# numamma/numamma

Measured on AMD Instinct MI355X. Metric: PEBS samples/s analysed (device-resident), higher is better.
Workload: dtype u64

## Files before the change

### numamma_amd/csrc/nmg_engine_impl.h

```cpp
#pragma once

#include <dlfcn.h>
#include <hip/hip_runtime.h>
#include <rccl/rccl.h>
#include <rocprofiler-sdk-roctx/roctx.h>

#include <algorithm>
#include <chrono>
#include <cinttypes>
#include <functional>
#include <cstdio>
#include <cstdlib>
#include <cstddef>
#include <cstring>
#include <condition_variable>
#include <memory>
#include <mutex>
#include <string>
#include <thread>
#include <vector>

#include "nmg_buffer.h"
#include "nmg_kernels.h"
#include "nmg_route.h"
// ... 70 lines not shown
  DevBuf<DevEntry> own_chain;
  DevEntry* chain = nullptr;
  uint32_t K = 0, elevels = 0, nb_fences = 0, fence_log2 = 0, dir_log2 = 0;
};

struct RouteTable {
  bool ok = false;
  uint32_t nparts = 0;
  DevBuf<PartInfo> d_parts;
  DevBuf<uint64_t> d_pbounds;
  DevBuf<uint16_t> d_pdir;
  DevBuf<uint32_t> d_pdead;
  DevBuf<uint64_t> d_pe_keys;
  DevBuf<uint4> d_pe_nodes;
  DevBuf<uint4> d_pe_pnode;
  DevBuf<uint4> d_pe_old;
  DevBuf<uint32_t> d_pe_oinf;
  DevBuf<uint2> d_pe_info;
  DevBuf<uint4> d_pe_dir;
  DevBuf<uint32_t> d_pe_ids;
  DevBuf<uint32_t> d_pe_lrel;
  DevBuf<uint32_t> d_pe_cmap;
};

struct RoutePool {
  DevBuf<uint4> d_rec16;
  DevBuf<uint32_t> d_cmeta;
  DevBuf<unsigned long long> d_cmatch;
  DevBuf<uint32_t> d_clist;
  DevBuf<uint4> d_items;
  DevBuf<uint32_t> d_chunk0;
  DevBuf<uint32_t> d_used;
  DevBuf<uint32_t> d_pcnt;
  DevBuf<uint32_t> d_pbase;
  DevBuf<uint32_t> d_ctl;
  DevBuf<uint4> d_ovf16;
  DevBuf<unsigned long long> d_ovfx;
};

struct EntryTable {
  std::vector<uint64_t> hist_base;
  std::vector<uint64_t> npages;
  std::vector<uint64_t> buffer_size, entry_addr;
  std::vector<nmg_object> objects;
  std::vector<DevEntry> dev_entries;
  std::vector<uint32_t> sparse_entries;
  CellCursor cur;

  uint64_t cells() const { return cur.cells; }
  void resize(uint32_t E) {
    const size_t E0 = dev_entries.size();
    hist_base.resize(E, kHistSparse);
    npages.resize(E, 1);
    buffer_size.resize(E, 0);
    entry_addr.resize(E, 0);
    objects.resize(E, nmg_object{0, 0, 0, 0});
    dev_entries.resize(E, DevEntry{0, 0, 0, 0, kHistSparse, ~0u, 0, 0, 0, 0});
    for (size_t e = E0; e < E; e++) dev_entries[e].id = (uint32_t)e;
  }
  void truncate(uint32_t E, const CellCursor& c) {
    resize(E);
    sparse_entries.resize(c.nsparse);
    cur = c;
  }
  void describe(uint32_t id, const nmg_object& o) {
    objects[id] = o;
    buffer_size[id] = o.buffer_size;
    entry_addr[id] = o.buffer_addr;
// ... 276 lines not shown
```

### numamma_amd/csrc/nmg_route.h

```cpp
#pragma once

#include "nmg_kernels.h"

namespace nmg {

constexpr uint32_t kChunk = 64;
constexpr uint32_t kPartLevels = 11;
constexpr uint32_t kMaxParts = (1u << kPartLevels) - 1;
constexpr uint32_t kRouteDir = 4096;
constexpr uint32_t kRouteSegs = 8;
constexpr uint32_t kDirCntSat = 31;
struct RSeg {
  uint64_t start;
  uint32_t base;
  uint32_t nslots;
  uint32_t shift;
  uint32_t qlast;
};
constexpr uint32_t kPartKeys = 1023;
constexpr uint32_t kPartSlots = 1024;
constexpr uint32_t kPartDir = 1024;
constexpr uint32_t kDirInline = 6;
constexpr uint32_t kPnQShift = 8;
constexpr uint32_t kPnOlder = 1u << 11, kPnExact = 1u << 12;
// ... 29 lines not shown
  uint32_t pages_lds;
  uint32_t cmap;
  uint32_t pad[2];
};
static_assert(sizeof(PartInfo) == 48, "PartInfo");

constexpr uint32_t kAddrBits = 40;
constexpr uint32_t kMinWeightBits = 11;
constexpr uint32_t kTsBits = 40;
struct XLayout {
  uint32_t gbits, obits, tbits, wbits;
  uint64_t wesc;
  uint64_t tbase;
};

struct RouteParams {
  Params p;
  const uint64_t* pbounds;
  const uint16_t* pdir;
  const uint32_t* pdead;
  RSeg seg[kRouteSegs];
  uint32_t nseg;
  uint32_t nparts;
  XLayout xl;
  uint64_t seq0;
  uint4* rec16;
  uint32_t* cmeta;
  const uint32_t* chunk0;
  uint32_t* used;
  uint4* ovf16;
  unsigned long long* ovfx;
  uint32_t* ovf_cnt;
  uint32_t ovf_cap;
};

struct PlanParams {
  uint32_t* pcnt;
  uint32_t* pbase;
  uint4* items;
  uint32_t* ctl;
  uint32_t grid, nparts;
};

struct ScatterParams {
  const uint32_t* cmeta;
  const uint32_t* chunk0;
  const uint32_t* used;
  const uint32_t* pcnt;
  const uint32_t* pbase;
  uint32_t* clist;
  uint32_t nparts;
};

struct LocalParams {
  Params p;
  const PartInfo* parts;
  const uint64_t* pe_keys;
  const uint4* pe_nodes;
  const uint4* pe_pnode;
  const uint4* pe_old;
  const uint32_t* pe_oinf;
  const uint2* pe_info;
  const uint4* pe_dir;
  const uint32_t* pe_ids;
  const uint32_t* pe_lrel;
  const uint32_t* pe_cmap;
  const uint4* rec16;
  const uint32_t* cmeta;
  const uint32_t* clist;
  const uint4* items;
  uint32_t* ctl;
  unsigned long long* cmatch;
  const BufDesc* descs;
  XLayout xl;
  uint64_t seq0;
  uint32_t fresh;
};

struct FoundParams {
  const uint32_t* ranges;
  const uint32_t* chunk0;
  const uint32_t* used;
  const uint32_t* cmeta;
  const unsigned long long* cmatch;
  const uint4* rec16;
  uint32_t* bufcnt;
  uint32_t nb_bufs, gbits, gshift;
};

hipError_t launch_route(uint32_t grid, hipStream_t s, const RouteParams& r);
hipError_t launch_overflow(hipStream_t s, const RouteParams& r);
struct CountParams {
  ScatterParams sc;
};
hipError_t launch_count(uint32_t grid, hipStream_t s, const CountParams& r);
hipError_t launch_plan(hipStream_t s, const PlanParams& r);
hipError_t launch_scatter(uint32_t grid, hipStream_t s, const ScatterParams& r);
hipError_t launch_local(uint32_t grid, hipStream_t s, const LocalParams& r);
hipError_t launch_found(uint32_t grid, hipStream_t s, const FoundParams& r);

}
```

### numamma_amd/csrc/nmg_route.hip

```cpp
#include <algorithm>

#include "nmg_device.h"
#include "nmg_route.h"

namespace nmg {

static_assert((uint64_t)kItemChunks * kChunk * kLaneMaxWeight < (1ull << kPackShift), "packed weight per item");


struct XRec {
  uint64_t addr, ts, w;
  uint64_t loc;
  uint32_t th, acc;
  bool esc;
  __device__ __forceinline__ uint32_t g(const XLayout& xl) const { return uint32_t(loc >> xl.obits); }
  __device__ __forceinline__ uint32_t off(const XLayout& xl) const {
    return uint32_t(loc & ((1ull << xl.obits) - 1)) << 3;
  }
};

__device__ __forceinline__ uint4 x_encode(const XLayout& xl, uint64_t pb, uint64_t addr, uint64_t ts, uint64_t w,
                                          uint32_t g, uint32_t off, uint32_t th, uint32_t acc) {
  const uint64_t ar = addr - pb, tr = ts - xl.tbase;
  const bool fit = (ar >> kAddrBits) == 0 && ts >= xl.tbase && (tr >> kTsBits) == 0 && w < xl.wesc;
// ... 321 lines not shown
__device__ __forceinline__ Claim route2_settle(uint64_t old, uint32_t q, unsigned long long* s_state, uint32_t& taken,
                                               uint32_t capl, uint32_t* cmeta, uint32_t c0) {
  Claim r;
  r.dst = ~0ull;
  r.lid = 0;
  r.waitg = 0;
  r.ovf = false;
  r.ok = true;
  const uint32_t f = st_cnt(old), g = st_gen(old), cu = st_cur(old), nx = st_next(old);
  if (cu != kStNone && f < 2 * kChunk) {
    const uint32_t c = f < kChunk ? cu : nx;
    if (c == kStOvf) r.ovf = true;
    else r.dst = uint64_t(c0 + c) * kChunk + (f & (kChunk - 1));
    r.lid = ((g << 6) + f) >> 2;
    if (f == kChunk + kChunk / 2) {
      const uint32_t n2 = route2_take(taken, capl);
      if (n2 != kStOvf) cmeta[c0 + n2] = q | (kChunk << 24);
      route2_advance(&s_state[q], g, n2, n2, false, old + 1);
    }
  } else if (cu == kStNone && f == 2 * kChunk) {
    const uint32_t n1 = route2_take(taken, capl);
    const uint32_t n2 = n1 == kStOvf ? kStOvf : route2_take(taken, capl);
    if (n1 != kStOvf) cmeta[c0 + n1] = q | (kChunk << 24);
    if (n2 != kStOvf) cmeta[c0 + n2] = q | (kChunk << 24);
    route2_advance(&s_state[q], g, n1, n2, true, old + 1);
    if (n1 == kStOvf) r.ovf = true;
    else r.dst = uint64_t(c0 + n1) * kChunk;
    r.lid = (g + 1) << 4;
  } else {
    r.waitg = g;
    r.ok = false;
  }
  return r;
}

struct XF {
  uint4 a;
  uint32_t q;
  uint32_t lvl;
  bool routed;
};

template <bool TIMING>
__global__ __launch_bounds__(kR2WG, 1) void route2_kernel(RouteParams rp) {
  __shared__ uint64_t s_pb[kMaxParts + 1];
  __shared__ uint16_t s_pdir[kRouteDir];
  __shared__ uint32_t s_dead[(kMaxParts + 1) / 32];
  __shared__ unsigned long long s_state[kMaxParts + 1];
  __shared__ uint4 s_desc[kDescLds];
  __shared__ uint32_t s_wlist[kWaves][64];
  __shared__ uint32_t s_taken, s_bnext;
  __shared__ unsigned long long s_gsums[2][kGlobalSums], s_gmins[2][kBuckets], s_gmaxs[2][kBuckets];
  __shared__ SegL s_seg[kRouteSegs];
  __shared__ uint64_t s_segst[kRouteSegs];
  __shared__ uint4 s_line[kLineParts * 4];
  __shared__ LineWord s_lw[kLineParts];
  __shared__ uint32_t s_ldst[kLineParts];
  __shared__ uint2 s_tab[kWaves][64];

  Params& p = rp.p;
  const int tid = threadIdx.x;
  const int lane = tid & 63, wave = tid >> 6;
  if (tid < (int)kRouteSegs) {
    const RSeg g = rp.seg[tid];
    s_seg[tid].a = make_uint4((uint32_t)g.start, (uint32_t)(g.start >> 32), g.base, g.nslots);
    s_seg[tid].b = make_uint4(g.shift, g.qlast, 0, 0);
// ... 320 lines not shown
            if (xr.esc) x_resolve(xr, rp.xl, p.data, p.sbufs);
            direct_attribute(p, xr.addr, xr.ts, xr.w, xr.th, xr.acc, X.lvl, rp.seq0 + xr.g(rp.xl), xr.off(rp.xl),
                             xr.g(rp.xl));
          }
        }
        vm_drain();
      }
      rt_stamp<TIMING>(rt, 10);
    };

    XF X;
    do {
      front(ra, rb, X);
      back(X);
      front(rb, ra, X);
      back(X);
    } while (d0.pad != kNoBuf);

    if (TIMING && lane == 0) {
      unsigned long long* o = p.dbg + (uint64_t(blockIdx.x) * (kWG / 64) + tid / 64) * kRouteTimingWords;
      for (int k = 0; k < 9; k++) o[k] = rt.acc[k];
      o[9] = nwin;
      uint32_t nb = 0;
      if (wave == 0)
        for (uint32_t q = 0; q < nlp; q++) nb += (s_lw[q] & kLwBroken) ? 1u : 0u;
      o[10] = nb;
      o[11] = rt.acc[9];
      o[12] = rt.acc[10];
    }
  }
  racc_drain(gacc[0], s_gsums[0], lane);
  racc_drain(gacc[1], s_gsums[1], lane);
  lds_sync();
#pragma unroll
  for (uint32_t a = 0; a < 2; a++) {
    if (tid < (int)kGlobalSums && s_gsums[a][tid])
      atomicAdd(reinterpret_cast<unsigned long long*>(p.sum64 + gsum_index(a, tid)), s_gsums[a][tid]);
    if (tid < (int)kBuckets && s_gsums[a][3 + 2 * tid]) {
      atomicMin(reinterpret_cast<unsigned long long*>(p.min64 + a * kBuckets + tid), s_gmins[a][tid]);
      atomicMax(reinterpret_cast<unsigned long long*>(p.max64 + a * kBuckets + tid), s_gmaxs[a][tid]);
    }
  }
  for (uint32_t q = tid; q < P; q += kR2WG) {
    const unsigned long long st = s_state[q];
    const uint32_t f = st_cnt(st), cu = st_cur(st), nx = st_next(st);
    if (cu == kStNone) continue;
    if (cu != kStOvf) rp.cmeta[c0 + cu] = q | (min(f, kChunk) << 24);
    if (nx != kStOvf) rp.cmeta[c0 + nx] = q | ((f > kChunk ? f - kChunk : 0u) << 24);
    if (q < nlp) {
      const uint32_t m = lw_mask(s_lw[q]);
      for (uint32_t j = 0; j < 4; j++)
        if ((m >> j) & 1u) rp.rec16[uint64_t(s_ldst[q]) * 4 + j] = s_line[q * 4 + j];
    }
  }
  if (tid == 0) rp.used[blockIdx.x] = min(s_taken, capl);
}


__global__ __launch_bounds__(256) void overflow_kernel(RouteParams rp) {
  const uint32_t n = min(*rp.ovf_cnt, rp.ovf_cap);
  for (uint32_t i = blockIdx.x * 256 + threadIdx.x; i < n; i += gridDim.x * 256) {
    XRec xr = x_decode(rp.xl, rp.ovfx[i], rp.ovf16[i]);
    if (xr.esc) x_resolve(xr, rp.xl, rp.p.data, rp.p.sbufs);
    const uint32_t lvl = (rp.p.flags & NMG_F_OBJECT_LEVELS)
                             ? raw_mem_lvl(rp.p.data, rp.p.sbufs[xr.g(rp.xl)].offset + xr.off(rp.xl))
                             : 0u;
    direct_attribute(rp.p, xr.addr, xr.ts, xr.w, xr.th, xr.acc, lvl, rp.seq0 + xr.g(rp.xl), xr.off(rp.xl),
                     xr.g(rp.xl));
  }
}


__global__ __launch_bounds__(kWG) void count_kernel(CountParams cp) {
  __shared__ uint32_t s_cnt[kMaxParts + 1];
  const ScatterParams& r = cp.sc;
  const uint32_t tid = threadIdx.x, w = blockIdx.x, P = r.nparts;
  for (uint32_t q = tid; q < P; q += kWG) s_cnt[q] = 0;
  __syncthreads();
  const uint32_t c0 = r.chunk0[w], n = r.used[w];
  constexpr uint32_t kU = 8;
  for (uint32_t b = 0; b < n; b += kU * kWG) {
    uint32_t m[kU];
#pragma unroll
    for (uint32_t u = 0; u < kU; u++) {
      const uint32_t i = b + u * kWG + tid;
      m[u] = i < n ? r.cmeta[c0 + i] : 0u;
    }
#pragma unroll
    for (uint32_t u = 0; u < kU; u++)
      if (m[u] >> 24) atomicAdd(&s_cnt[m[u] & 0xffffffu], 1u);
  }
  __syncthreads();
  uint32_t* out = const_cast<uint32_t*>(r.pcnt) + uint64_t(w) * P;
  for (uint32_t q = tid; q < P; q += kWG) out[q] = s_cnt[q];
}

constexpr uint32_t kPlanRowGroups = kWG / 64;
__global__ __launch_bounds__(kWG) void plan_cols_kernel(PlanParams r) {
  __shared__ uint32_t s_sum[kPlanRowGroups][64];
  const uint32_t tid = threadIdx.x, c = tid & 63, rg = tid >> 6;
  const uint32_t P = r.nparts, q = blockIdx.x * 64 + c;
  const uint32_t per = (r.grid + kPlanRowGroups - 1) / kPlanRowGroups, w0 = rg * per;
  constexpr uint32_t kU = 16;
  uint32_t sum = 0;
  for (uint32_t b = 0; b < per; b += kU) {
    uint32_t v[kU];
#pragma unroll
    for (uint32_t u = 0; u < kU; u++) {
      const uint32_t w = w0 + b + u;
      v[u] = (q < P && b + u < per && w < r.grid) ? r.pcnt[uint64_t(w) * P + q] : 0u;
    }
#pragma unroll
    for (uint32_t u = 0; u < kU; u++) sum += v[u];
  }
  s_sum[rg][c] = sum;
  __syncthreads();
  uint32_t run = 0;
  for (uint32_t g = 0; g < rg; g++) run += s_sum[g][c];
  for (uint32_t b = 0; b < per; b += kU) {
    uint32_t v[kU];
#pragma unroll
    for (uint32_t u = 0; u < kU; u++) {
      const uint32_t w = w0 + b + u;
      v[u] = (q < P && b + u < per && w < r.grid) ? r.pcnt[uint64_t(w) * P + q] : 0u;
    }
#pragma unroll
    for (uint32_t u = 0; u < kU; u++) {
      const uint32_t w = w0 + b + u;
      if (q < P && b + u < per && w < r.grid) r.pcnt[uint64_t(w) * P + q] = run;
      run += v[u];
    }
  }
  if (q < P && rg == kPlanRowGroups - 1) r.pbase[q] = run;
}

__global__ __launch_bounds__(kWG) void plan_kernel(PlanParams r) {
  __shared__ uint32_t s_tot[kMaxParts + 1], s_nit[kMaxParts + 1], s_wsum[2][kWG / 64];
  const int tid = threadIdx.x, lane = tid & 63, wave = tid >> 6;
  const uint32_t P = r.nparts;
  for (uint32_t q = tid; q < P; q += kWG) {
    const uint32_t run = r.pbase[q];
    s_tot[q] = run;
    s_nit[q] = (run + kItemChunks - 1) / kItemChunks;
  }
  __syncthreads();
  const uint32_t i0 = 2 * (uint32_t)tid;
  const uint32_t t0 = i0 < P ? s_tot[i0] : 0u, t1 = i0 + 1 < P ? s_tot[i0 + 1] : 0u;
  const uint32_t n0 = i0 < P ? s_nit[i0] : 0u, n1 = i0 + 1 < P ? s_nit[i0 + 1] : 0u;
  uint32_t it = t0 + t1, in = n0 + n1;
#pragma unroll
  for (int o = 1; o < 64; o <<= 1) {
    const uint32_t a = __shfl_up(it, o, 64), b = __shfl_up(in, o, 64);
    if (lane >= o) {
      it += a;
      in += b;
    }
  }
  if (lane == 63) {
    s_wsum[0][wave] = it;
    s_wsum[1][wave] = in;
  }
  __syncthreads();
  uint32_t wt = 0, wn = 0;
  for (int w2 = 0; w2 < wave; w2++) {
    wt += s_wsum[0][w2];
    wn += s_wsum[1][w2];
  }
  const uint32_t tb = wt + it - (t0 + t1), nb = wn + in - (n0 + n1);
  for (uint32_t k = 0; k < 2; k++) {
    const uint32_t q = i0 + k;
    if (q >= P) break;
    const uint32_t base = tb + (k ? t0 : 0u), ibase = nb + (k ? n0 : 0u), tot = k ? t1 : t0;
    r.pbase[q] = base;
    for (uint32_t j = 0; j * kItemChunks < tot; j++)
      r.items[ibase + j] = make_uint4(q, base + j * kItemChunks, base + min(tot, (j + 1) * kItemChunks),
                                      tot <= kItemChunks ? 1u : 0u);
  }
  if (tid == kWG - 1) {
    r.ctl[0] = wn + in;
    r.ctl[1] = 0;
    r.ctl[3] = r.ctl[2];
    r.ctl[2] = 0;
  }
}

__global__ __launch_bounds__(kWG) void scatter_kernel(ScatterParams r) {
  __shared__ uint32_t s_cnt[kMaxParts + 1];
  const uint32_t tid = threadIdx.x, w = blockIdx.x, P = r.nparts;
  const uint32_t* off = r.pcnt + uint64_t(w) * P;
  for (uint32_t q = tid; q < P; q += kWG) s_cnt[q] = r.pbase[q] + off[q];
  __syncthreads();
  const uint32_t c0 = r.chunk0[w], n = r.used[w];
  constexpr uint32_t kU = 8;
  for (uint32_t b = 0; b < n; b += kU * kWG) {
    uint32_t m[kU];
#pragma unroll
    for (uint32_t u = 0; u < kU; u++) {
      const uint32_t i = b + u * kWG + tid;
      m[u] = i < n ? r.cmeta[c0 + i] : 0u;
    }
#pragma unroll
    for (uint32_t u = 0; u < kU; u++) {
      if (!(m[u] >> 24)) continue;
      const uint32_t k = atomicAdd(&s_cnt[m[u] & 0xffffffu], 1u);
      r.clist[k] = (c0 + b + u * kWG + tid) | ((m[u] >> 24) << kChunkIdBits);
    }
  }
}


constexpr uint32_t kLWG = 1024;
constexpr int kLC = 2;

template <typename T>
__device__ __forceinline__ T l2_load(const T* p) {
  return __hip_atomic_load(p, __ATOMIC_RELAXED, __HIP_MEMORY_SCOPE_AGENT);
}

__device__ __forceinline__ uint64_t entry_id(const LocalParams& lp, uint32_t pos) {
  return lp.pe_ids ? lp.pe_ids[pos] : pos;
}

__device__ __forceinline__ int32_t match_older_pos(const Params& p, uint32_t first, uint32_t count, uint64_t addr,
                                                   uint64_t ts, uint64_t& baddr, uint64_t& hist) {
  for (uint32_t j = first + 1; j < first + count; j++) {
    const uint4* r = reinterpret_cast<const uint4*>(p.chain + j);
    const uint4 ra = r[0], rb = r[1];
    if (entry_match(ra, rb, addr, ts)) {
      const uint4 rc = r[2];
      baddr = u64of(ra.x, ra.y);
      hist = u64of(rc.x, rc.y);
      return (int32_t)j;
    }
  }
  return -1;
}

template <bool TIMING, bool PACKED, bool EXTRA>
__global__ __launch_bounds__(kLWG, 1) void local_kernel(LocalParams lp) {
  __shared__ uint64_t s_keys[kPartSlots];
  __shared__ uint4 s_pn[kPartSlots];
  __shared__ uint2 s_info[kPartSlots];
  __shared__ uint4 s_dir[kPartDir];
  __shared__ uint4 s_old[kOldLds];
  __shared__ uint32_t s_oinf[kOldLds];
  __shared__ unsigned long long s_owt[2][kPartEntries];
  __shared__ unsigned long long s_first[kPartEntries];
  __shared__ uint32_t s_pg[kPartCells / 2];
  __shared__ uint32_t s_clist[kItemChunks];
  __shared__ uint32_t s_item, s_cnext, s_nfound, s_big, s_took;
// ... 414 lines not shown
        if (TIMING) {
          const uint64_t now = stamp();
          textra += now - rt.last;
          rt.last = now;
        }
      }
    };
    uint4 A[kLC], B[kLC];
    auto grab = [&]() -> uint32_t {
      uint32_t t = 0;
      if (lane == 0) t = atomicAdd(&s_cnext, (uint32_t)kLC);
      return __builtin_amdgcn_readfirstlane(t);
    };
    uint32_t la = grab(), lb = grab();
#pragma unroll
    for (int j = 0; j < kLC; j++) chunk_load(la + j, A[j]);
#pragma unroll
    for (int j = 0; j < kLC; j++) chunk_load(lb + j, B[j]);
    while (la < nl) {
      process(la, A);
      la = grab();
#pragma unroll
      for (int j = 0; j < kLC; j++) chunk_load(la + j, A[j]);
      if (lb < nl) process(lb, B);
      lb = grab();
#pragma unroll
      for (int j = 0; j < kLC; j++) chunk_load(lb + j, B[j]);
    }
    uint32_t won = 0;
    if (lane == 0) won = atomicExch(&s_took, 1u) == 0 ? 1u : 0u;
    if (__builtin_amdgcn_readfirstlane(won)) take_next();
    lds_sync();
    rt_stamp<TIMING>(rt, 9);
    const bool clean =excl && lp.fresh && __builtin_amdgcn_readfirstlane(lp.ctl[3]) == 0;
    const bool clean_obj = clean && __builtin_amdgcn_readfirstlane(s_big) == 0;
    for (uint32_t i = tid; i < pi.ne; i += kLWG) {
      const uint64_t e = entry_id(lp, pi.e0 + i);
#pragma unroll
      for (uint32_t a = 0; a < 2; a++) {
        const uint64_t v = s_owt[a][i];
        if (!v) continue;
        s_owt[a][i] = 0;
        const uint64_t cnt = v >> kPackShift, wt = v & ((1ull << kPackShift) - 1);
        uint64_t* pc = p.sum64 + objcw_index(e, a, 0, p.nb_entries);
        uint64_t* pw = p.sum64 + objcw_index(e, a, 1, p.nb_entries);
        if (clean_obj) {
          *pc = cnt;
          if (wt) *pw = wt;
        } else if (excl) {
          *pc = l2_load(pc) + cnt;
          if (wt) *pw = l2_load(pw) + wt;
        } else {
          atomicAdd(reinterpret_cast<unsigned long long*>(pc), (unsigned long long)cnt);
          if (wt) atomicAdd(reinterpret_cast<unsigned long long*>(pw), (unsigned long long)wt);
        }
      }
      const uint64_t floc = s_first[i];
      if (floc != ~0ull) {
        s_first[i] = ~0ull;
        const uint64_t fo = ((lp.seq0 + (floc >> lp.xl.obits)) << 32) | ((floc & ((1ull << lp.xl.obits) - 1)) << 3);
        uint64_t* pf = p.min64 + kFirstBase + e;
        if (clean) *pf = fo;
        else if (excl) *pf = min(l2_load(pf), fo);
        else atomicMin(reinterpret_cast<unsigned long long*>(pf), (unsigned long long)fo);
      }
    }
    {
// ... 56 lines not shown
  for (uint32_t i = tid; i < nl; i += kWG) s_found[i] = 0;
  __syncthreads();
  const uint64_t k0 = uint64_t(r.chunk0[w]) * kChunk, k1 = k0 + uint64_t(r.used[w]) * kChunk;
  const uint64_t gmask = (1ull << r.gbits) - 1;
  constexpr int kU = 4;
  for (uint64_t k = k0 + tid; k < k1; k += kU * kWG) {
    uint64_t bits[kU], xw[kU];
#pragma unroll
    for (int u = 0; u < kU; u++) {
      const uint64_t kk = k + u * kWG;
      bits[u] = kk < k1 && (r.cmeta[kk / kChunk] >> 24) ? r.cmatch[kk / kChunk] : 0ull;
      xw[u] = ((bits[u] >> lane) & 1) ? reinterpret_cast<const uint64_t*>(r.rec16)[2 * kk + 1] >> r.gshift : 0ull;
    }
#pragma unroll
    for (int u = 0; u < kU; u++) {
      if (!((bits[u] >> lane) & 1)) continue;
      const uint32_t g = (uint32_t)(xw[u] & gmask);
      if (g - g0 < nl) atomicAdd(&s_found[g - g0], 1u);
      else atomicAdd(r.bufcnt + r.nb_bufs + g, 1u);
    }
  }
  __syncthreads();
  for (uint32_t i = tid; i < nl; i += kWG)
    if (s_found[i]) atomicAdd(r.bufcnt + r.nb_bufs + g0 + i, s_found[i]);
}


hipError_t launch_route(uint32_t grid, hipStream_t s, const RouteParams& r) {
  if (r.p.flags & kDbgRouteTiming) hipLaunchKernelGGL(route2_kernel<true>, dim3(grid), dim3(kR2WG), 0, s, r);
  else hipLaunchKernelGGL(route2_kernel<false>, dim3(grid), dim3(kR2WG), 0, s, r);
  return hipGetLastError();
}

hipError_t launch_plan(hipStream_t s, const PlanParams& r) {
  if (r.nparts) hipLaunchKernelGGL(plan_cols_kernel, dim3((r.nparts + 63) / 64), dim3(kWG), 0, s, r);
  hipLaunchKernelGGL(plan_kernel, dim3(1), dim3(kWG), 0, s, r);
  return hipGetLastError();
}

hipError_t launch_overflow(hipStream_t s, const RouteParams& r) {
  hipLaunchKernelGGL(overflow_kernel, dim3(1024), dim3(256), 0, s, r);
  return hipGetLastError();
}

hipError_t launch_count(uint32_t grid, hipStream_t s, const CountParams& r) {
  hipLaunchKernelGGL(count_kernel, dim3(grid), dim3(kWG), 0, s, r);
  return hipGetLastError();
}

hipError_t launch_scatter(uint32_t grid, hipStream_t s, const ScatterParams& r) {
  hipLaunchKernelGGL(scatter_kernel, dim3(grid), dim3(kWG), 0, s, r);
  return hipGetLastError();
}

template <bool TIMING, bool PACKED>
static void launch_local_as(bool extra, uint32_t grid, hipStream_t s, const LocalParams& r) {
  if (extra) hipLaunchKernelGGL((local_kernel<TIMING, PACKED, true>), dim3(grid), dim3(kLWG), 0, s, r);
  else hipLaunchKernelGGL((local_kernel<TIMING, PACKED, false>), dim3(grid), dim3(kLWG), 0, s, r);
}

hipError_t launch_local(uint32_t grid, hipStream_t s, const LocalParams& r) {
  const bool timing = (r.p.flags & kDbgLocalTiming) != 0, packed = r.pe_cmap != nullptr;
  const bool extra = (r.p.flags & NMG_F_OBJECT_LEVELS) != 0 || r.p.smatch != nullptr;
  if (packed) {
    if (timing) launch_local_as<true, true>(extra, grid, s, r);
    else launch_local_as<false, true>(extra, grid, s, r);
  } else {
    if (timing) launch_local_as<true, false>(extra, grid, s, r);
    else launch_local_as<false, false>(extra, grid, s, r);
  }
  return hipGetLastError();
}

hipError_t launch_found(uint32_t grid, hipStream_t s, const FoundParams& r) {
  hipLaunchKernelGGL(found_kernel, dim3(grid), dim3(kWG), 0, s, r);
  return hipGetLastError();
}

}
```

### numamma_amd/csrc/nmg_route_host.hip

```cpp
#include "nmg_engine_impl.h"


uint32_t bits_for(uint64_t v) {
  uint32_t b = 0;
  while (b < 64 && (v >> b) != 0) b++;
  return b;
}

bool route_layout(nmg_engine* h, const std::vector<BufDesc>& descs, XLayout& xl) {
  uint64_t maxlen = 1;
  for (const BufDesc& d : descs) maxlen = std::max<uint64_t>(maxlen, d.len);
  xl.gbits = bits_for(descs.size() - 1);
  xl.obits = bits_for((maxlen - 1) / 8);
  xl.tbits = bits_for(h->T - 1);
  const uint32_t loc = xl.gbits + xl.obits + xl.tbits + 1;
  if (loc > 48 - kMinWeightBits || xl.gbits > 31 || xl.obits > 31 || xl.tbits > 31) return false;
  xl.wbits = std::min<uint32_t>(48 - loc, 16);
  xl.wesc = (1ull << xl.wbits) - 1;
  xl.tbase = h->route_tbase;
  return true;
}

bool route_eligible(nmg_engine* h, const std::vector<BufDesc>& descs) {
  constexpr uint32_t kLegacyOnly = kDbgLoadOnly | kDbgNoGlobal | kDbgNoFlush | kDbgNoTables | kDbgTiming |
// ... 12 lines not shown
bool route_eligible(nmg_engine* h) { return route_eligible(h, h->descs); }

int route_pool(nmg_engine* h, const std::vector<BufDesc>& descs, uint32_t grid, const uint32_t* ranges,
                      std::vector<uint32_t>& c0) {
  const uint32_t P = h->rt.nparts;
  c0.assign(grid + 1, 0);
  uint64_t tot = 0;
  for (uint32_t w = 0; w < grid; w++) {
    uint64_t rec = 0;
    for (uint32_t b = ranges[w]; b < ranges[w + 1]; b++) rec += (descs[b].len + kRecBytes - 1) / kRecBytes;
    const uint64_t cap = (h->flags & kDbgTinyPool) ? 2 : (rec + kChunk - 1) / kChunk + 2 * P;
    c0[w] = (uint32_t)tot;
    tot += cap;
  }
  c0[grid] = (uint32_t)tot;
  if (tot >= (1ull << kChunkIdBits)) return fail(h, NMG_ERR_RANGE, "partition-first chunk pool too large");
  const size_t items = tot / kItemChunks + P + 1;
  uint64_t recs = 0;
  for (const BufDesc& d : descs) recs += (d.len + kRecBytes - 1) / kRecBytes;
  const size_t ovf = (size_t)((h->flags & kDbgTinyPool) ? recs : recs / 4 + std::min<uint64_t>(3 * recs, 4u << 20)) + 65536;
  RoutePool& rp = h->rpool;
  if (tot > rp.d_cmeta.cap() || items > rp.d_items.cap() || grid > rp.d_used.cap() || ovf > rp.d_ovfx.cap()) {
    HIP_TRY(h, hipStreamSynchronize(h->stream));
    rp = RoutePool();
    const size_t cap = std::max<size_t>(tot, 1);
    HIP_TRY(h, rp.d_rec16.alloc(cap * kChunk));
    HIP_TRY(h, rp.d_cmeta.alloc(cap));
    HIP_TRY(h, rp.d_cmatch.alloc(cap));
    HIP_TRY(h, rp.d_clist.alloc(cap));
    HIP_TRY(h, rp.d_items.alloc(items));
    HIP_TRY(h, rp.d_chunk0.alloc(grid + 1));
    HIP_TRY(h, rp.d_used.alloc(grid));
    HIP_TRY(h, rp.d_pcnt.alloc((size_t)grid * (kMaxParts + 1)));
    HIP_TRY(h, rp.d_pbase.alloc(kMaxParts + 1));
    HIP_TRY(h, rp.d_ctl.alloc(4));
    HIP_TRY(h, hipMemset(rp.d_ctl, 0, 4 * 4));
    HIP_TRY(h, rp.d_ovf16.alloc(ovf));
    HIP_TRY(h, rp.d_ovfx.alloc(ovf));
  }
  return NMG_OK;
}

int route_prepare(nmg_engine* h, uint32_t grid, const std::vector<uint32_t>& ranges) {
  std::vector<uint32_t> c0;
  const int rc = route_pool(h, h->descs, grid, ranges.data(), c0);
  if (rc) return rc;
  const int rc2 = stage_h2d(h, h->rpool.d_chunk0, c0.data(), (grid + 1) * 4);
  if (rc2) return rc2;
  h->route_sched_key = h->rt.nparts | ((h->flags & kDbgTinyPool) ? 0x80000000u : 0u);
  return NMG_OK;
}


int route_analyze(nmg_engine* h, uint32_t nb, uint32_t grid) {
  (void)nb;
  RouteJob job{&h->descs, h->d_data, h->d_sdescs, h->d_ranges, h->rpool.d_chunk0, grid, 0, false};
  return route_analyze_job(h, job);
}

int route_analyze_job(nmg_engine* h, const RouteJob& job) {
  Range range("nmg_route");
  XLayout xl;
  if (!route_layout(h, *job.descs, xl)) return fail(h, NMG_ERR_STATE, "route layout");
  const uint32_t grid = job.grid;
  Params base = base_params(h, job.data, job.sdescs, job.ranges);
  base.bufcnt = h->d_bufcnt + job.index_base;
  const uint64_t seq0 = (*job.descs)[0].seq;
  h->route_launches++;
  int slot = 0;
  int rc = launch_events(h, &slot);
  if (rc) return rc;
  HIP_TRY(h, hipEventRecord(h->ring0[slot], h->stream));
  RouteParams rp;
  memset(&rp, 0, sizeof(rp));
  rp.p = base;
  rp.pbounds = h->rt.d_pbounds;
  rp.pdir = h->rt.d_pdir;
  rp.pdead = h->rt.d_pdead;
  for (uint32_t k = 0; k < kRouteSegs; k++) rp.seg[k] = h->rsegs[k];
  rp.nseg = h->nrsegs;
  rp.nparts = h->rt.nparts;
  rp.xl = xl;
  rp.seq0 = seq0;
  rp.rec16 = h->rpool.d_rec16;
  rp.cmeta = h->rpool.d_cmeta;
  rp.chunk0 = job.chunk0;
  rp.used = h->rpool.d_used;
  rp.ovf16 = h->rpool.d_ovf16;
  rp.ovfx = h->rpool.d_ovfx;
  rp.ovf_cnt = h->rpool.d_ctl + 2;
  rp.ovf_cap = (uint32_t)std::min<size_t>(h->rpool.d_ovfx.cap(), 0xffffffffu);
  if (h->flags & kDbgTinyOvf) rp.ovf_cap = std::min<uint32_t>(rp.ovf_cap, 64);
  if (h->flags & kDbgRouteTiming) {
    rc = ensure_dbg(h, (size_t)grid * (kWG / 64) * kRouteTimingWords);
    if (rc) return rc;
    rp.p.dbg = reinterpret_cast<unsigned long long*>(h->d_dbg.get());
  }
  HIP_TRY(h, launch_route(grid, h->stream, rp));
  HIP_TRY(h, hipEventRecord(h->ringr[slot], h->stream));
  HIP_TRY(h, launch_overflow(h->stream, rp));
  ScatterParams sc;
  sc.cmeta = h->rpool.d_cmeta;
  sc.chunk0 = job.chunk0;
  sc.used = h->rpool.d_used;
  sc.pcnt = h->rpool.d_pcnt;
  sc.pbase = h->rpool.d_pbase;
  sc.clist = h->rpool.d_clist;
  sc.nparts = h->rt.nparts;
  CountParams cp;
  memset(&cp, 0, sizeof(cp));
  cp.sc = sc;
  HIP_TRY(h, launch_count(grid, h->stream, cp));
  PlanParams pl;
  pl.pcnt = h->rpool.d_pcnt;
  pl.pbase = h->rpool.d_pbase;
  pl.items = h->rpool.d_items;
  pl.ctl = h->rpool.d_ctl;
  pl.grid = grid;
  pl.nparts = h->rt.nparts;
  HIP_TRY(h, launch_plan(h->stream, pl));
  HIP_TRY(h, launch_scatter(grid, h->stream, sc));
  LocalParams lp;
  memset(&lp, 0, sizeof(lp));
  lp.p = base;
  lp.parts = h->rt.d_parts;
  lp.pe_keys = h->rt.d_pe_keys;
  lp.pe_nodes = h->rt.d_pe_nodes;
  lp.pe_info = h->rt.d_pe_info;
  lp.pe_pnode = h->rt.d_pe_pnode;
  lp.pe_old = h->rt.d_pe_old;
  lp.pe_oinf = h->rt.d_pe_oinf;
  lp.pe_dir = h->rt.d_pe_dir;
  lp.pe_ids = h->rt.d_pe_ids;
  lp.pe_lrel = h->rt.d_pe_lrel;
  lp.pe_cmap = h->rt.d_pe_cmap;
  lp.rec16 = h->rpool.d_rec16;
  lp.cmeta = h->rpool.d_cmeta;
  lp.clist = h->rpool.d_clist;
  lp.items = h->rpool.d_items;
  lp.ctl = h->rpool.d_ctl;
  lp.cmatch = h->rpool.d_cmatch;
  lp.descs = job.sdescs;
  lp.xl = xl;
  lp.seq0 = seq0;
  lp.fresh = h->counters_fresh ? 1u : 0u;
  h->counters_fresh = false;
  if ((h->flags & kDbgLocalTiming) && !(h->flags & kDbgRouteTiming)) {
    rc = ensure_dbg(h, (size_t)h->num_cus * (kWG / 64) * kRouteTimingWords);
    if (rc) return rc;
    lp.p.dbg = reinterpret_cast<unsigned long long*>(h->d_dbg.get());
  }
  HIP_TRY(h, launch_local((uint32_t)h->num_cus, h->stream, lp));
  HIP_TRY(h, hipEventRecord(h->ringm[slot], h->stream));
  HIP_TRY(h, hipEventRecord(h->ring1[slot], h->stream));
  h->nlaunch++;
  h->launched = true;
  if (job.settle_now) {
    FoundParams f;
    f.ranges = job.ranges;
    f.chunk0 = job.chunk0;
    f.used = h->rpool.d_used;
    f.cmeta = h->rpool.d_cmeta;
    f.cmatch = h->rpool.d_cmatch;
    f.rec16 = h->rpool.d_rec16;
    f.bufcnt = h->d_bufcnt + job.index_base;
    f.nb_bufs = (uint32_t)h->bufcnt_stride;
    f.gbits = xl.gbits;
    f.gshift = 16 + xl.wbits + xl.obits;
    HIP_TRY(h, launch_found(grid, h->stream, f));
    return NMG_OK;
  }
  h->route_pending = true;
  h->route_grid = grid;
// ... 23 lines not shown
```

Before: 45.76 billion.

## Fold count and plan into route/scatter kernels with atomic partition totals

The route kernel now counts per-partition chunks itself, right after writing cmeta, and reserves per-block offsets with agent-scope atomic adds on a partition-total array. The scatter kernel absorbs the overflow handling, the item-plan scan and the per-block base computation, so four separate launches (overflow, count, plan_cols, plan) disappear. Double-buffered totals and overflow counters, selected by launch parity, are reset for the next launch from inside scatter. The cost is that per-block offsets now depend on atomic ordering instead of a deterministic column scan. It also adds redundant scan work in every scatter block and a cmeta re-read with a drain and barrier in route.

```diff
diff --git a/numamma_amd/csrc/nmg_engine_impl.h b/numamma_amd/csrc/nmg_engine_impl.h
--- a/numamma_amd/csrc/nmg_engine_impl.h
+++ b/numamma_amd/csrc/nmg_engine_impl.h
@@ -126,8 +126,9 @@
   DevBuf<uint32_t> d_chunk0;
   DevBuf<uint32_t> d_used;
   DevBuf<uint32_t> d_pcnt;
-  DevBuf<uint32_t> d_pbase;
+  DevBuf<uint32_t> d_ptot;
   DevBuf<uint32_t> d_ctl;
+  uint32_t launches = 0;
   DevBuf<uint4> d_ovf16;
   DevBuf<unsigned long long> d_ovfx;
 };
diff --git a/numamma_amd/csrc/nmg_route.h b/numamma_amd/csrc/nmg_route.h
--- a/numamma_amd/csrc/nmg_route.h
+++ b/numamma_amd/csrc/nmg_route.h
@@ -85,14 +85,8 @@
   unsigned long long* ovfx;
   uint32_t* ovf_cnt;
   uint32_t ovf_cap;
-};
-
-struct PlanParams {
+  uint32_t* ptot;
   uint32_t* pcnt;
-  uint32_t* pbase;
-  uint4* items;
-  uint32_t* ctl;
-  uint32_t grid, nparts;
 };
 
 struct ScatterParams {
@@ -100,8 +94,12 @@
   const uint32_t* chunk0;
   const uint32_t* used;
   const uint32_t* pcnt;
-  const uint32_t* pbase;
+  const uint32_t* ptot;
+  uint32_t* ptot_next;
+  uint32_t* ovf_next;
   uint32_t* clist;
+  uint4* items;
+  uint32_t* ctl;
   uint32_t nparts;
 };
 
@@ -123,6 +121,7 @@
   const uint32_t* clist;
   const uint4* items;
   uint32_t* ctl;
+  const uint32_t* ovf_cnt;
   unsigned long long* cmatch;
   const BufDesc* descs;
   XLayout xl;
@@ -142,13 +141,7 @@
 };
 
 hipError_t launch_route(uint32_t grid, hipStream_t s, const RouteParams& r);
-hipError_t launch_overflow(hipStream_t s, const RouteParams& r);
-struct CountParams {
-  ScatterParams sc;
-};
-hipError_t launch_count(uint32_t grid, hipStream_t s, const CountParams& r);
-hipError_t launch_plan(hipStream_t s, const PlanParams& r);
-hipError_t launch_scatter(uint32_t grid, hipStream_t s, const ScatterParams& r);
+hipError_t launch_scatter(uint32_t grid, hipStream_t s, const RouteParams& r, const ScatterParams& sc);
 hipError_t launch_local(uint32_t grid, hipStream_t s, const LocalParams& r);
 hipError_t launch_found(uint32_t grid, hipStream_t s, const FoundParams& r);
 
diff --git a/numamma_amd/csrc/nmg_route.hip b/numamma_amd/csrc/nmg_route.hip
--- a/numamma_amd/csrc/nmg_route.hip
+++ b/numamma_amd/csrc/nmg_route.hip
@@ -377,6 +377,11 @@
     r.ok = false;
   }
   return r;
+}
+
+template <typename T>
+__device__ __forceinline__ T l2_load(const T* p) {
+  return __hip_atomic_load(p, __ATOMIC_RELAXED, __HIP_MEMORY_SCOPE_AGENT);
 }
 
 struct XF {
@@ -763,6 +768,8 @@
   racc_drain(gacc[0], s_gsums[0], lane);
   racc_drain(gacc[1], s_gsums[1], lane);
   lds_sync();
+  uint32_t* s_cnt = reinterpret_cast<uint32_t*>(s_pb);
+  for (uint32_t q = tid; q < P; q += kR2WG) s_cnt[q] = 0;
 #pragma unroll
   for (uint32_t a = 0; a < 2; a++) {
     if (tid < (int)kGlobalSums && s_gsums[a][tid])
@@ -784,13 +791,37 @@
         if ((m >> j) & 1u) rp.rec16[uint64_t(s_ldst[q]) * 4 + j] = s_line[q * 4 + j];
     }
   }
-  if (tid == 0) rp.used[blockIdx.x] = min(s_taken, capl);
-}
-
-
-__global__ __launch_bounds__(256) void overflow_kernel(RouteParams rp) {
-  const uint32_t n = min(*rp.ovf_cnt, rp.ovf_cap);
-  for (uint32_t i = blockIdx.x * 256 + threadIdx.x; i < n; i += gridDim.x * 256) {
+  const uint32_t nused = __builtin_amdgcn_readfirstlane(min(s_taken, capl));
+  if (tid == 0) rp.used[blockIdx.x] = nused;
+  vm_drain();
+  __syncthreads();
+  constexpr uint32_t kTU = 4;
+  for (uint32_t b = 0; b < nused; b += kTU * kR2WG) {
+    uint32_t m[kTU];
+#pragma unroll
+    for (uint32_t u = 0; u < kTU; u++) {
+      const uint32_t i = b + u * kR2WG + tid;
+      m[u] = i < nused ? l2_load(rp.cmeta + c0 + i) : 0u;
+    }
+#pragma unroll
+    for (uint32_t u = 0; u < kTU; u++)
+      if (m[u] >> 24) atomicAdd(&s_cnt[m[u] & 0xffffffu], 1u);
+  }
+  lds_sync();
+  uint32_t* out = rp.pcnt + uint64_t(blockIdx.x) * P;
+  for (uint32_t q = tid; q < P; q += kR2WG) {
+    const uint32_t n = s_cnt[q];
+    out[q] = n ? __hip_atomic_fetch_add(rp.ptot + q, n, __ATOMIC_RELAXED, __HIP_MEMORY_SCOPE_AGENT) : 0u;
+  }
+}
+
+static_assert(2 * kWG >= kMaxParts + 1, "scatter_kernel scans two partitions per thread");
+__global__ __launch_bounds__(kWG) void scatter_kernel(RouteParams rp, ScatterParams r) {
+  __shared__ uint32_t s_cnt[kMaxParts + 1];
+  __shared__ uint32_t s_wsum[2][kWG / 64];
+  const uint32_t tid = threadIdx.x, lane = tid & 63, wave = tid >> 6, w = blockIdx.x, P = r.nparts;
+  const uint32_t novf = min(*rp.ovf_cnt, rp.ovf_cap);
+  for (uint32_t i = w * kWG + tid; i < novf; i += gridDim.x * kWG) {
     XRec xr = x_decode(rp.xl, rp.ovfx[i], rp.ovf16[i]);
     if (xr.esc) x_resolve(xr, rp.xl, rp.p.data, rp.p.sbufs);
     const uint32_t lvl = (rp.p.flags & NMG_F_OBJECT_LEVELS)
@@ -799,14 +830,50 @@
     direct_attribute(rp.p, xr.addr, xr.ts, xr.w, xr.th, xr.acc, lvl, rp.seq0 + xr.g(rp.xl), xr.off(rp.xl),
                      xr.g(rp.xl));
   }
-}
-
-
-__global__ __launch_bounds__(kWG) void count_kernel(CountParams cp) {
-  __shared__ uint32_t s_cnt[kMaxParts + 1];
-  const ScatterParams& r = cp.sc;
-  const uint32_t tid = threadIdx.x, w = blockIdx.x, P = r.nparts;
-  for (uint32_t q = tid; q < P; q += kWG) s_cnt[q] = 0;
+  const uint32_t* off = r.pcnt + uint64_t(w) * P;
+  const uint32_t i0 = 2 * tid;
+  const uint32_t t0 = i0 < P ? r.ptot[i0] : 0u, t1 = i0 + 1 < P ? r.ptot[i0 + 1] : 0u;
+  const uint32_t o0 = i0 < P ? off[i0] : 0u, o1 = i0 + 1 < P ? off[i0 + 1] : 0u;
+  const uint32_t n0 = (t0 + kItemChunks - 1) / kItemChunks, n1 = (t1 + kItemChunks - 1) / kItemChunks;
+  uint32_t it = t0 + t1, in = n0 + n1;
+#pragma unroll
+  for (int o = 1; o < 64; o <<= 1) {
+    const uint32_t a = __shfl_up(it, o, 64), b = __shfl_up(in, o, 64);
+    if (lane >= (uint32_t)o) {
+      it += a;
+      in += b;
+    }
+  }
+  if (lane == 63) {
+    s_wsum[0][wave] = it;
+    s_wsum[1][wave] = in;
+  }
+  __syncthreads();
+  uint32_t wt = 0, wn = 0;
+  for (uint32_t w2 = 0; w2 < wave; w2++) {
+    wt += s_wsum[0][w2];
+    wn += s_wsum[1][w2];
+  }
+  const uint32_t tb = wt + it - (t0 + t1), nb = wn + in - (n0 + n1);
+  if (i0 < P) s_cnt[i0] = tb + o0;
+  if (i0 + 1 < P) s_cnt[i0 + 1] = tb + t0 + o1;
+  if (w == 0) {
+    for (uint32_t k = 0; k < 2; k++) {
+      const uint32_t q = i0 + k;
+      if (q >= P) break;
+      const uint32_t base = tb + (k ? t0 : 0u), ibase = nb + (k ? n0 : 0u), tot = k ? t1 : t0;
+      for (uint32_t j = 0; j * kItemChunks < tot; j++)
+        r.items[ibase + j] = make_uint4(q, base + j * kItemChunks, base + min(tot, (j + 1) * kItemChunks),
+                                        tot <= kItemChunks ? 1u : 0u);
+    }
+    r.ptot_next[i0] = 0;
+    r.ptot_next[i0 + 1] = 0;
+    if (tid == kWG - 1) {
+      r.ctl[0] = wn + in;
+      r.ctl[1] = 0;
+      *r.ovf_next = 0;
+    }
+  }
   __syncthreads();
   const uint32_t c0 = r.chunk0[w], n = r.used[w];
   constexpr uint32_t kU = 8;
@@ -818,119 +885,6 @@
       m[u] = i < n ? r.cmeta[c0 + i] : 0u;
     }
 #pragma unroll
-    for (uint32_t u = 0; u < kU; u++)
-      if (m[u] >> 24) atomicAdd(&s_cnt[m[u] & 0xffffffu], 1u);
-  }
-  __syncthreads();
-  uint32_t* out = const_cast<uint32_t*>(r.pcnt) + uint64_t(w) * P;
-  for (uint32_t q = tid; q < P; q += kWG) out[q] = s_cnt[q];
-}
-
-constexpr uint32_t kPlanRowGroups = kWG / 64;
-__global__ __launch_bounds__(kWG) void plan_cols_kernel(PlanParams r) {
-  __shared__ uint32_t s_sum[kPlanRowGroups][64];
-  const uint32_t tid = threadIdx.x, c = tid & 63, rg = tid >> 6;
-  const uint32_t P = r.nparts, q = blockIdx.x * 64 + c;
-  const uint32_t per = (r.grid + kPlanRowGroups - 1) / kPlanRowGroups, w0 = rg * per;
-  constexpr uint32_t kU = 16;
-  uint32_t sum = 0;
-  for (uint32_t b = 0; b < per; b += kU) {
-    uint32_t v[kU];
-#pragma unroll
-    for (uint32_t u = 0; u < kU; u++) {
-      const uint32_t w = w0 + b + u;
-      v[u] = (q < P && b + u < per && w < r.grid) ? r.pcnt[uint64_t(w) * P + q] : 0u;
-    }
-#pragma unroll
-    for (uint32_t u = 0; u < kU; u++) sum += v[u];
-  }
-  s_sum[rg][c] = sum;
-  __syncthreads();
-  uint32_t run = 0;
-  for (uint32_t g = 0; g < rg; g++) run += s_sum[g][c];
-  for (uint32_t b = 0; b < per; b += kU) {
-    uint32_t v[kU];
-#pragma unroll
-    for (uint32_t u = 0; u < kU; u++) {
-      const uint32_t w = w0 + b + u;
-      v[u] = (q < P && b + u < per && w < r.grid) ? r.pcnt[uint64_t(w) * P + q] : 0u;
-    }
-#pragma unroll
-    for (uint32_t u = 0; u < kU; u++) {
-      const uint32_t w = w0 + b + u;
-      if (q < P && b + u < per && w < r.grid) r.pcnt[uint64_t(w) * P + q] = run;
-      run += v[u];
-    }
-  }
-  if (q < P && rg == kPlanRowGroups - 1) r.pbase[q] = run;
-}
-
-__global__ __launch_bounds__(kWG) void plan_kernel(PlanParams r) {
-  __shared__ uint32_t s_tot[kMaxParts + 1], s_nit[kMaxParts + 1], s_wsum[2][kWG / 64];
-  const int tid = threadIdx.x, lane = tid & 63, wave = tid >> 6;
-  const uint32_t P = r.nparts;
-  for (uint32_t q = tid; q < P; q += kWG) {
-    const uint32_t run = r.pbase[q];
-    s_tot[q] = run;
-    s_nit[q] = (run + kItemChunks - 1) / kItemChunks;
-  }
-  __syncthreads();
-  const uint32_t i0 = 2 * (uint32_t)tid;
-  const uint32_t t0 = i0 < P ? s_tot[i0] : 0u, t1 = i0 + 1 < P ? s_tot[i0 + 1] : 0u;
-  const uint32_t n0 = i0 < P ? s_nit[i0] : 0u, n1 = i0 + 1 < P ? s_nit[i0 + 1] : 0u;
-  uint32_t it = t0 + t1, in = n0 + n1;
-#pragma unroll
-  for (int o = 1; o < 64; o <<= 1) {
-    const uint32_t a = __shfl_up(it, o, 64), b = __shfl_up(in, o, 64);
-    if (lane >= o) {
-      it += a;
-      in += b;
-    }
-  }
-  if (lane == 63) {
-    s_wsum[0][wave] = it;
-    s_wsum[1][wave] = in;
-  }
-  __syncthreads();
-  uint32_t wt = 0, wn = 0;
-  for (int w2 = 0; w2 < wave; w2++) {
-    wt += s_wsum[0][w2];
-    wn += s_wsum[1][w2];
-  }
-  const uint32_t tb = wt + it - (t0 + t1), nb = wn + in - (n0 + n1);
-  for (uint32_t k = 0; k < 2; k++) {
-    const uint32_t q = i0 + k;
-    if (q >= P) break;
-    const uint32_t base = tb + (k ? t0 : 0u), ibase = nb + (k ? n0 : 0u), tot = k ? t1 : t0;
-    r.pbase[q] = base;
-    for (uint32_t j = 0; j * kItemChunks < tot; j++)
-      r.items[ibase + j] = make_uint4(q, base + j * kItemChunks, base + min(tot, (j + 1) * kItemChunks),
-                                      tot <= kItemChunks ? 1u : 0u);
-  }
-  if (tid == kWG - 1) {
-    r.ctl[0] = wn + in;
-    r.ctl[1] = 0;
-    r.ctl[3] = r.ctl[2];
-    r.ctl[2] = 0;
-  }
-}
-
-__global__ __launch_bounds__(kWG) void scatter_kernel(ScatterParams r) {
-  __shared__ uint32_t s_cnt[kMaxParts + 1];
-  const uint32_t tid = threadIdx.x, w = blockIdx.x, P = r.nparts;
-  const uint32_t* off = r.pcnt + uint64_t(w) * P;
-  for (uint32_t q = tid; q < P; q += kWG) s_cnt[q] = r.pbase[q] + off[q];
-  __syncthreads();
-  const uint32_t c0 = r.chunk0[w], n = r.used[w];
-  constexpr uint32_t kU = 8;
-  for (uint32_t b = 0; b < n; b += kU * kWG) {
-    uint32_t m[kU];
-#pragma unroll
-    for (uint32_t u = 0; u < kU; u++) {
-      const uint32_t i = b + u * kWG + tid;
-      m[u] = i < n ? r.cmeta[c0 + i] : 0u;
-    }
-#pragma unroll
     for (uint32_t u = 0; u < kU; u++) {
       if (!(m[u] >> 24)) continue;
       const uint32_t k = atomicAdd(&s_cnt[m[u] & 0xffffffu], 1u);
@@ -942,11 +896,6 @@
 
 constexpr uint32_t kLWG = 1024;
 constexpr int kLC = 2;
-
-template <typename T>
-__device__ __forceinline__ T l2_load(const T* p) {
-  return __hip_atomic_load(p, __ATOMIC_RELAXED, __HIP_MEMORY_SCOPE_AGENT);
-}
 
 __device__ __forceinline__ uint64_t entry_id(const LocalParams& lp, uint32_t pos) {
   return lp.pe_ids ? lp.pe_ids[pos] : pos;
@@ -1427,7 +1376,7 @@
     if (__builtin_amdgcn_readfirstlane(won)) take_next();
     lds_sync();
     rt_stamp<TIMING>(rt, 9);
-    const bool clean =excl && lp.fresh && __builtin_amdgcn_readfirstlane(lp.ctl[3]) == 0;
+    const bool clean =excl && lp.fresh && __builtin_amdgcn_readfirstlane(*lp.ovf_cnt) == 0;
     const bool clean_obj = clean && __builtin_amdgcn_readfirstlane(s_big) == 0;
     for (uint32_t i = tid; i < pi.ne; i += kLWG) {
       const uint64_t e = entry_id(lp, pi.e0 + i);
@@ -1550,24 +1499,8 @@
   return hipGetLastError();
 }
 
-hipError_t launch_plan(hipStream_t s, const PlanParams& r) {
-  if (r.nparts) hipLaunchKernelGGL(plan_cols_kernel, dim3((r.nparts + 63) / 64), dim3(kWG), 0, s, r);
-  hipLaunchKernelGGL(plan_kernel, dim3(1), dim3(kWG), 0, s, r);
-  return hipGetLastError();
-}
-
-hipError_t launch_overflow(hipStream_t s, const RouteParams& r) {
-  hipLaunchKernelGGL(overflow_kernel, dim3(1024), dim3(256), 0, s, r);
-  return hipGetLastError();
-}
-
-hipError_t launch_count(uint32_t grid, hipStream_t s, const CountParams& r) {
-  hipLaunchKernelGGL(count_kernel, dim3(grid), dim3(kWG), 0, s, r);
-  return hipGetLastError();
-}
-
-hipError_t launch_scatter(uint32_t grid, hipStream_t s, const ScatterParams& r) {
-  hipLaunchKernelGGL(scatter_kernel, dim3(grid), dim3(kWG), 0, s, r);
+hipError_t launch_scatter(uint32_t grid, hipStream_t s, const RouteParams& r, const ScatterParams& sc) {
+  hipLaunchKernelGGL(scatter_kernel, dim3(grid), dim3(kWG), 0, s, r, sc);
   return hipGetLastError();
 }
 
diff --git a/numamma_amd/csrc/nmg_route_host.hip b/numamma_amd/csrc/nmg_route_host.hip
--- a/numamma_amd/csrc/nmg_route_host.hip
+++ b/numamma_amd/csrc/nmg_route_host.hip
@@ -68,7 +68,8 @@
     HIP_TRY(h, rp.d_chunk0.alloc(grid + 1));
     HIP_TRY(h, rp.d_used.alloc(grid));
     HIP_TRY(h, rp.d_pcnt.alloc((size_t)grid * (kMaxParts + 1)));
-    HIP_TRY(h, rp.d_pbase.alloc(kMaxParts + 1));
+    HIP_TRY(h, rp.d_ptot.alloc(2 * (kMaxParts + 1)));
+    HIP_TRY(h, hipMemset(rp.d_ptot, 0, 2 * (kMaxParts + 1) * 4));
     HIP_TRY(h, rp.d_ctl.alloc(4));
     HIP_TRY(h, hipMemset(rp.d_ctl, 0, 4 * 4));
     HIP_TRY(h, rp.d_ovf16.alloc(ovf));
@@ -124,7 +125,10 @@
   rp.used = h->rpool.d_used;
   rp.ovf16 = h->rpool.d_ovf16;
   rp.ovfx = h->rpool.d_ovfx;
-  rp.ovf_cnt = h->rpool.d_ctl + 2;
+  const uint32_t par = h->rpool.launches & 1u;
+  rp.ovf_cnt = h->rpool.d_ctl + 2 + par;
+  rp.ptot = h->rpool.d_ptot + (size_t)par * (kMaxParts + 1);
+  rp.pcnt = h->rpool.d_pcnt;
   rp.ovf_cap = (uint32_t)std::min<size_t>(h->rpool.d_ovfx.cap(), 0xffffffffu);
   if (h->flags & kDbgTinyOvf) rp.ovf_cap = std::min<uint32_t>(rp.ovf_cap, 64);
   if (h->flags & kDbgRouteTiming) {
@@ -132,30 +136,23 @@
     if (rc) return rc;
     rp.p.dbg = reinterpret_cast<unsigned long long*>(h->d_dbg.get());
   }
+  h->rpool.launches++;
   HIP_TRY(h, launch_route(grid, h->stream, rp));
   HIP_TRY(h, hipEventRecord(h->ringr[slot], h->stream));
-  HIP_TRY(h, launch_overflow(h->stream, rp));
   ScatterParams sc;
+  memset(&sc, 0, sizeof(sc));
   sc.cmeta = h->rpool.d_cmeta;
   sc.chunk0 = job.chunk0;
   sc.used = h->rpool.d_used;
   sc.pcnt = h->rpool.d_pcnt;
-  sc.pbase = h->rpool.d_pbase;
+  sc.ptot = rp.ptot;
+  sc.ptot_next = h->rpool.d_ptot + (size_t)(par ^ 1u) * (kMaxParts + 1);
+  sc.ovf_next = h->rpool.d_ctl + 2 + (par ^ 1u);
   sc.clist = h->rpool.d_clist;
+  sc.items = h->rpool.d_items;
+  sc.ctl = h->rpool.d_ctl;
   sc.nparts = h->rt.nparts;
-  CountParams cp;
-  memset(&cp, 0, sizeof(cp));
-  cp.sc = sc;
-  HIP_TRY(h, launch_count(grid, h->stream, cp));
-  PlanParams pl;
-  pl.pcnt = h->rpool.d_pcnt;
-  pl.pbase = h->rpool.d_pbase;
-  pl.items = h->rpool.d_items;
-  pl.ctl = h->rpool.d_ctl;
-  pl.grid = grid;
-  pl.nparts = h->rt.nparts;
-  HIP_TRY(h, launch_plan(h->stream, pl));
-  HIP_TRY(h, launch_scatter(grid, h->stream, sc));
+  HIP_TRY(h, launch_scatter(grid, h->stream, rp, sc));
   LocalParams lp;
   memset(&lp, 0, sizeof(lp));
   lp.p = base;
@@ -175,6 +172,7 @@
   lp.clist = h->rpool.d_clist;
   lp.items = h->rpool.d_items;
   lp.ctl = h->rpool.d_ctl;
+  lp.ovf_cnt = rp.ovf_cnt;
   lp.cmatch = h->rpool.d_cmatch;
   lp.descs = job.sdescs;
   lp.xl = xl;
```

Result: no change. 46.19 billion (median of 6 runs) (+0.9%).
